# kaiidams/Kokoro-Align

Hardware: NVIDIA B200
Metric: lattice cells/sec (TxS) (higher is better)
Workload: dtype f32

## Files before the change

kokoro-align_b200/csrc/kab_api.cu:

```cuda
#include "../../include/kokoro_align_b200.h"

#include <algorithm>
#include <atomic>
#include <chrono>
#include <map>
#include <mutex>
#include <thread>
#include <unordered_map>
#include <cstdio>
#include <cstdlib>
#include <cstring>
#include <functional>
#include <limits>
#include <new>
#include <optional>
#include <vector>

#include "kab_band.cuh"
#include "kab_bandp.cuh"
#include "kab_bandr.cuh"
#include "kab_btpar.cuh"
#include "kab_wide.cuh"
#include "kab_common.cuh"
#include "kab_compact.cuh"
// ... 195 lines not shown
    if (se.first == stream) ev = se.second;
  if (!ev) {
    KAB_CUDA(cudaEventCreateWithFlags(&ev, cudaEventDisableTiming));
    pl->run_events.emplace_back(stream, ev);
  }
  KAB_CUDA(cudaEventRecord(ev, stream));
  return KAB_OK;
}

void host_teardown(kab_plan *pl) {
  for (kab_plan *c : pl->segs) plan_free(c);
  pl->segs.clear();
  pl->seg_b0.clear();
  for (int k = 0; k < kab_plan::NPIPE; ++k) {
    if (pl->pipe[k]) plan_free(pl->pipe[k]);
    pl->pipe[k] = nullptr;
    pl->pipe_rows[k].clear();
    if (pl->ev_pipe_in[k]) cudaEventDestroy(pl->ev_pipe_in[k]);
    if (pl->ev_pipe_done[k]) cudaEventDestroy(pl->ev_pipe_done[k]);
    if (pl->s_pipe[k]) cudaStreamDestroy(pl->s_pipe[k]);
    pl->ev_pipe_in[k] = nullptr; pl->ev_pipe_done[k] = nullptr; pl->s_pipe[k] = nullptr;
  }
  for (cudaEvent_t e : pl->ev_in) cudaEventDestroy(e);
  for (cudaEvent_t e : pl->ev_cmp) cudaEventDestroy(e);
  pl->ev_in.clear();
  pl->ev_cmp.clear();
  pool_free(pl->d_lp); pool_free(pl->d_path); pool_free(pl->d_lab); pool_free(pl->d_st);
  pool_free(pl->d_sc); pool_free(pl->d_fs); pool_free(pl->d_seg_off); pool_free(pl->d_seg_rec); pool_free(pl->d_lab8);
  pl->d_lp = nullptr; pl->d_path = nullptr; pl->d_lab = nullptr; pl->d_st = nullptr;
  pl->d_sc = nullptr; pl->d_fs = nullptr; pl->d_seg_off = nullptr; pl->d_seg_rec = nullptr; pl->d_lab8 = nullptr;
  pl->seg_cap = 0;
  if (pl->stream) cudaStreamDestroy(pl->stream);
  if (pl->s_in) cudaStreamDestroy(pl->s_in);
  if (pl->s_out) cudaStreamDestroy(pl->s_out);
  pl->stream = nullptr; pl->s_in = nullptr; pl->s_out = nullptr;
  pl->host_ready = false;
}

int plan_free(kab_plan *pl) {
  if (!pl) return KAB_OK;
  Trace tr("kab_plan_destroy");
  DeviceGuard guard;
  guard.enter(pl->device);
  for (auto &se : pl->run_events) {
    cudaEventSynchronize(se.second);
    cudaEventDestroy(se.second);
  }
  pl->run_events.clear();
  if (pl->stream) cudaStreamSynchronize(pl->stream);
  if (pl->s_out) cudaStreamSynchronize(pl->s_out);
  host_teardown(pl);
  if (pl->s_sub) cudaStreamSynchronize(pl->s_sub);
  if (pl->sub) plan_free(pl->sub);
  if (pl->ev_fork) cudaEventDestroy(pl->ev_fork);
  if (pl->ev_join) cudaEventDestroy(pl->ev_join);
  if (pl->s_sub) cudaStreamDestroy(pl->s_sub);
  for (int q = 0; q < N_QUEUES; ++q) pool_free(pl->d_lists[q]);
  pool_free(pl->d_col16); pool_free(pl->d_raw); pool_free(pl->d_bp); pool_free(pl->d_scratch);
  pool_free(pl->d_queue); pool_free(pl->d_status_init); pool_free(pl->d_wide_ws); pool_free(pl->d_band_fifo); pool_free(pl->d_bt_meta); pool_free(pl->d_bt_maps); pool_free(pl->d_bt_entry); pool_free(pl->d_end_state); pool_free(pl->d_gather); pool_free(pl->d_lpc); pool_free(pl->d_nonfinite); pool_free(pl->d_t_off); pool_free(pl->d_seg_scratch); pool_free(pl->d_started);
  delete pl;
  tr.mark("free");
  return KAB_OK;
}

}

extern "C" {

int kab_version(void) { return KAB_VERSION; }

const char *kab_error_string(int code) {
  switch (code) {
    case KAB_OK: return "ok";
    case KAB_E_CUDA: return "CUDA error (see kab_last_cuda_error)";
    case KAB_E_BAD_ARG: return "bad argument";
    case KAB_E_NOMEM: return "out of host memory";
    case KAB_E_UNSUPPORTED: return "unsupported shape";
    default: return "unknown error";
  }
}

const char *kab_last_cuda_error(void) { return g_cuda_err; }

int kab_device_count(int *count) {
  if (!count) return KAB_E_BAD_ARG;
  KAB_CUDA(cudaGetDeviceCount(count));
  return KAB_OK;
}

namespace {
int plan_create_impl(kab_plan **out, int device, const PlanSpec &s, int64_t B, const int64_t *t_off,
                     const int32_t *labels, const int64_t *l_off, const uint8_t *mask, int band_mode);
constexpr int32_t CTC_W = 0x3fffffff, CTC_M = 3;
constexpr int64_t CTC_BAND_MAX_W = 3264;
}

int kab_plan_create(kab_plan **out, int device, int64_t B, const int64_t *t_off, const int32_t *labels,
                    const int64_t *l_off, int32_t V, int32_t W, int32_t M) {
  return plan_create_impl(out, device, PlanSpec{V, W, M}, B, t_off, labels, l_off, nullptr, -1);
}

int kab_plan_create_ctc(kab_plan **out, int device, int64_t B, const int64_t *t_off, const int32_t *labels,
                        const int64_t *l_off, int32_t V, int32_t blank) {
  if (blank < 0 || blank >= V) return KAB_E_BAD_ARG;
  return plan_create_impl(out, device, PlanSpec{V, CTC_W, CTC_M, true, blank}, B, t_off, labels, l_off, nullptr, 0);
}

int kab_plan_create_ctc_long(kab_plan **out, int device, int64_t B, const int64_t *t_off, const int32_t *labels,
                             const int64_t *l_off, int32_t V, int32_t blank) {
  if (blank < 0 || blank >= V) return KAB_E_BAD_ARG;
  return plan_create_impl(out, device, PlanSpec{V, CTC_W, CTC_M, true, blank, true}, B, t_off, labels, l_off, nullptr, 0);
}

int kab_plan_create_ctc_band(kab_plan **out, int device, int64_t B, const int64_t *t_off, const int32_t *labels,
                             const int64_t *l_off, int32_t V, int32_t blank, int32_t beam_size) {
  if (blank < 0 || blank >= V || beam_size < 1) return KAB_E_BAD_ARG;
  return plan_create_impl(out, device, PlanSpec{V, beam_size, CTC_M, true, blank, true}, B, t_off, labels, l_off, nullptr, 0);
}

namespace {

struct Knobs {
  int stage_frames, band_cluster, band_q, band_r, band_hybrid, serial_bt, warp_ctas_per_sm;
  bool band_gather, ctc_compact, serial_setup;
  static int get(const char *name) { const char *v = getenv(name); return v ? atoi(v) : -1; }
  static Knobs read() {
    const char *sb = getenv("KAB_BAND_SERIAL_BT");
    return Knobs{get("KAB_STAGE_FRAMES"), get("KAB_BAND_CLUSTER"), get("KAB_BAND_Q"), get("KAB_BAND_R"), get("KAB_BAND_HYBRID"),
                 sb ? (atoi(sb) != 0) : -1, get("KAB_WARP_CTAS_PER_SM"), get("KAB_BAND_GATHER") != 0, get("KAB_CTC_COMPACT") != 0,
                 getenv("KAB_SERIAL_SETUP") != nullptr};
  }
};

struct LatFacts { uint8_t bad, special, compact; int32_t distinct, repeats; int64_t col_off; };

struct Setup {
  kab_plan *pl;
  const PlanSpec &s;
  const Knobs knob;
  int64_t B;
  const int64_t *t_off, *l_off;
  const int32_t *labels;
  const uint8_t *mask;
  bool gather = false;
  int32_t Veff = 0;
  std::vector<LatFacts> facts;
  std::vector<int32_t> gather_rows;
  std::vector<uint16_t> col16;
  std::vector<int32_t> status_init;
  int64_t bp_bytes = 0, scr_floats = 0, max_band_weff = 0;
  int wide_capacity = 0, wide_max_ctas = 0;
  std::vector<uint8_t> hyb_mask;
  int hyb_k = 0;
  bool in(int64_t b) const { return !mask || mask[b]; }
  int64_t frames(int64_t b) const { return t_off[b + 1] - t_off[b]; }
  int64_t len(int64_t b) const { return l_off[b + 1] - l_off[b]; }
  void for_lattices(const std::function<void(int64_t, int64_t *)> &fn) const;
  void scan_labels(), compact_vocabulary(), classify(), choose_band_kernel(int band_mode), lay_out_band();
  int allocate(), finish();
};

void Setup::for_lattices(const std::function<void(int64_t, int64_t *)> &fn) const {
  const int n_mask = (s.V + 63) / 64;
  const unsigned hw = std::thread::hardware_concurrency();
  const int nt = (B >= 2048 && pl->total_L >= 65536 && hw >= 4 && !knob.serial_setup) ? (int)std::min<unsigned>(8, hw / 2) : 1;
  auto work = [&](int t) {
    std::vector<int64_t> words((size_t)std::max(n_mask, 1), 0);
    const int64_t b0 = B * t / nt, b1 = B * (t + 1) / nt;
    for (int64_t b = b0; b < b1; ++b)
      if (in(b)) fn(b, words.data());
  };
  std::vector<std::thread> th;
  for (int t = 1; t < nt; ++t) th.emplace_back(work, t);
  work(0);
  for (auto &w : th) w.join();
}

void Setup::scan_labels() {
  const int n_mask = (s.V + 63) / 64;
  facts.assign((size_t)B, LatFacts{});
  for_lattices([&](int64_t b, int64_t *seen) {
    const int64_t L = len(b);
    const int32_t *lab = labels + l_off[b];
    LatFacts f{};
    std::fill(seen, seen + n_mask, (int64_t)0);
    for (int64_t l = 0; l < L; ++l) {
      if (s.ctc ? (lab[l] < 0 || lab[l] >= s.V || lab[l] == s.blank) : (lab[l] < -s.V || lab[l] >= s.V)) { f.bad = 1; break; }
      if (!s.ctc && lab[l] <= 0) f.special = 1;
      if (l > 0 && lab[l] == lab[l - 1]) ++f.repeats;
      const int32_t c = lab[l] < 0 ? lab[l] + s.V : lab[l];
      if (!(seen[c >> 6] >> (c & 63) & 1)) { seen[c >> 6] |= (int64_t)1 << (c & 63); ++f.distinct; }
    }
    facts[(size_t)b] = f;
  });
}

void Setup::compact_vocabulary() {
  const int64_t ga_max_weff = (int64_t)KAB_BQ_OW * KAB_BR_CW * 8 - 32;
  bool ok = !s.ctc && s.V > MAX_STAGE_V && s.M <= 4 && knob.band_gather && kab_bandr_geom(64).smem_bytes <= 227 * 1024, any_band = false;
  for (int64_t b = 0; b < B && ok; ++b) {
    const int64_t S = 2 * len(b) + 1;
    if (in(b) && band_shaped(frames(b), S, s.W)) { any_band = true; ok = std::min<int64_t>(s.W, S) <= ga_max_weff; }
  }
  gather = ok && any_band;
  int64_t dmax = -1, off = 0;
  for (int64_t b = 0; b < B; ++b) {
    if (!in(b)) continue;
    LatFacts &f = facts[(size_t)b];
    f.col_off = off;
    if (f.bad) continue;
    off += align_up(len(b), 8) + 8;
    if (f.special || (gather && band_shaped(frames(b), 2 * len(b) + 1, s.W))) continue;
    if (!s.ctc || f.distinct + 1 <= MAX_STAGE_V) dmax = std::max<int64_t>(dmax, f.distinct);
  }
  if (s.V > MAX_STAGE_V && (s.ctc ? knob.ctc_compact : s.M <= 4) && dmax >= 0 && dmax + 1 <= MAX_STAGE_V) {
    pl->Vc = (int32_t)std::max<int64_t>(8, align_up(dmax + 1, 4));
    gather_rows.assign((size_t)B * pl->Vc, 0);
  }
  Veff = pl->Vc ? pl->Vc : s.V;

  pl->stage_frames = Veff <= 64 ? 16 : 8;
  if (knob.stage_frames == 8 || knob.stage_frames == 16 || knob.stage_frames == 32) pl->stage_frames = knob.stage_frames;
  pl->stage_bytes = (int32_t)align_up((int64_t)pl->stage_frames * Veff * 4 + 24, 16);

  col16.assign((size_t)off, 0);
  const int n_mask = (s.V + 63) / 64;
  for_lattices([&](int64_t b, int64_t *seen) {
    LatFacts &f = facts[(size_t)b];
    if (f.bad) return;
    const int64_t L = len(b);
    const int32_t *lab = labels + l_off[b];
    uint16_t *c = col16.data() + f.col_off;
    const bool ga = gather && !f.special && band_shaped(frames(b), 2 * L + 1, s.W);
    if (pl->Vc && !f.special && !ga && f.distinct + 1 <= pl->Vc) {
      f.compact = 1;
      std::fill(seen, seen + n_mask, (int64_t)0);
      for (int64_t l = 0; l < L; ++l) seen[lab[l] >> 6] |= (int64_t)1 << (lab[l] & 63);
      int32_t *g = gather_rows.data() + (size_t)b * pl->Vc;
      g[0] = s.ctc ? s.blank : 0;
      int32_t n = 1;
      for (int w = 0; w < n_mask; ++w)
        for (int64_t m = seen[w]; m; m &= m - 1) g[n++] = w * 64 + __builtin_ctzll((unsigned long long)m);
      for (int64_t l = 0; l < L; ++l) c[l] = (uint16_t)(std::lower_bound(g + 1, g + n, lab[l]) - g);
    } else {
      for (int64_t l = 0; l < L; ++l) c[l] = (uint16_t)(lab[l] < 0 ? lab[l] + s.V : lab[l]);
    }
  });
}

void Setup::classify() {
  const int64_t W = s.W, M = s.M;
  Launch &lw = pl->launch[Q_WIDE];
  lw = Launch{s.ctc ? (const void *)kab_wide_ctc_kernel : (const void *)kab_wide_kernel, dim3(), dim3(KAB_WD_THREADS),
              kab_wide_geom(pl->stage_bytes).smem_bytes, 0, true};
  {
    int occ = 0;
    if (lw.smem <= 227 * 1024 && ensure_dyn_smem(lw.fn, pl->device, lw.smem) == cudaSuccess &&
        cudaOccupancyMaxActiveBlocksPerMultiprocessor(&occ, lw.fn, KAB_WD_THREADS, lw.smem) == cudaSuccess)
      wide_capacity = occ * pl->sm_count;
    (void)cudaGetLastError();
  }
  bool ctc_wide = false;
  if (s.ctc && s.ctc_long) {
    double sum_t = 0.0, cells = 0.0, max_cells = 0.0;
    for (int64_t b = 0; b < B; ++b) {
      if (!in(b) || facts[(size_t)b].bad) continue;
      if (pl->Vc && !facts[(size_t)b].compact) continue;
      const int64_t T = frames(b), S = 2 * len(b) + 1;
      if (!unbanded(T, S, W)) continue;
      if (S + 32 <= KAB_BAND_OW * BAND_MAX_WARPS) continue;
      if (wide_ctas(S) + 1 > wide_capacity) continue;
      sum_t += (double)T;
      cells += (double)T * (double)S;
      max_cells = std::max(max_cells, (double)T * (double)S);
    }
    ctc_wide = sum_t * 102.0 <= std::max(max_cells / 0.68, cells / 79.0);
  }
  kab_plan_info &info = pl->info;
  status_init.assign((size_t)B, 0);
  for (int64_t b = 0; b < B; ++b) {
    if (!in(b)) continue;
    const int64_t T = frames(b), L = len(b), S = 2 * L + 1;
    const LatFacts &f = facts[(size_t)b];
    if (f.bad || (s.ctc && T < L + f.repeats)) {
      status_init[(size_t)b] = f.bad ? KAB_ST_BAD_LABEL : KAB_ST_DEAD_BAND;
      pl->any_bad_label = true;
      continue;
    }
    KabLattice d{};
    d.t_off = t_off[b];
    d.lab_off = l_off[b];
    d.T = (int32_t)T; d.L = (int32_t)L; d.index = (int32_t)b;
    d.col_off = f.col_off;
    const bool ga = gather && !f.special && band_shaped(T, S, W);

    const bool fast = M <= 4 && !f.special && (ga || (Veff <= MAX_STAGE_V && (!pl->Vc || f.distinct + 1 <= pl->Vc)));
    const bool full = unbanded(T, S, W);
    const int64_t weff = std::min<int64_t>(W, S);
    int q;
    if (fast && !ga && full && S <= 248) {
      q = Q_WARP;
      d.k = S <= 62 ? 2 : (S <= 124 ? 4 : (S <= 186 ? 6 : 8));
      d.bp_off = bp_bytes;
      if (s.ctc || d.k <= 4) {
        const int fpw = d.k <= 2 ? 8 : (d.k <= 4 ? 4 : 2);
        bp_bytes += align_up((T + fpw - 1) / fpw * 128, 256);
      } else {
        bp_bytes += align_up((T + KAB_CKPT_C - 1) / KAB_CKPT_C * kab_ckpt_stride((int)S, d.k) * 4, 256);
      }
    } else if (fast && band_shaped(T, S, W) && (!s.ctc || full || weff <= CTC_BAND_MAX_W)) {
      q = Q_BAND;
      max_band_weff = std::max(max_band_weff, weff);
    } else if (fast && !ga && (s.ctc ? ctc_wide : M == 4) && full && wide_ctas(S) + 1 <= wide_capacity) {
      q = Q_WIDE;
      const int nww = (int)((S + KAB_BAND_OW - 1) / KAB_BAND_OW);
      d.k = nww;
      wide_max_ctas = std::max(wide_max_ctas, (int)wide_ctas(S));
      d.bp_off = bp_bytes;
      bp_bytes += (int64_t)nww * ((T + 7) / 8) * 256;
      d.scr_off = pl->wide_ws_bytes / 4;
      pl->wide_ws_bytes += (int64_t)align_up((int64_t)kab_wide_ws_bytes(nww), 256);
    } else {
      q = Q_GENERIC;
      d.bp_off = bp_bytes;
      bp_bytes += align_up(T * std::max<int64_t>(1, weff), 256);
      d.scr_off = scr_floats;
      scr_floats += align_up(2 * (S + 16), 64);
    }
    pl->lists[q].push_back(d);
    pl->max_T[q] = std::max(pl->max_T[q], (int)T);
    info.n_class[q == Q_WARP ? KAB_CLASS_WARP : (q == Q_GENERIC ? KAB_CLASS_GENERIC : (q == Q_WIDE ? KAB_CLASS_WIDE : KAB_CLASS_BAND))]++;
    const int64_t cells = cells_eval_of(T, S, W);
    info.cells_eval += cells;
    info.cells_nominal += T * S;
    int bbits = 0;
    while ((1 << bbits) < M) ++bbits;
    const int64_t dcols = std::min<int64_t>(s.V, f.distinct + 1);
    info.algorithmic_bytes += 4 * dcols * T + (cells * bbits + 7) / 8 + (T * bbits + 7) / 8 + 12 * T;
  }
}

void Setup::choose_band_kernel(int band_mode) {
  std::vector<KabLattice> &bl = pl->lists[Q_BAND];
  if (bl.empty()) return;
  pl->band_nw = (int32_t)((max_band_weff + 32 + KAB_BAND_OW - 1) / KAB_BAND_OW);
  const int nc = (pl->band_nw + KAB_BP_CW - 1) / KAB_BP_CW;
  int want_nc = knob.band_cluster;
  if (band_mode >= 0) want_nc = band_mode == 0 ? 0 : -1;
  const bool cluster_ok = nc <= 8 && kab_bandp_geom(pl->stage_bytes).smem_bytes <= 227 * 1024;
  const int nwq = (int)((max_band_weff + 32 + KAB_BQ_OW - 1) / KAB_BQ_OW);
  const int ncq = (nwq + KAB_BQ_CW - 1) / KAB_BQ_CW;
  const bool q_ok = ncq <= 8 && kab_bandq_geom(pl->stage_bytes).smem_bytes <= 227 * 1024;
  const int ncr = (nwq + KAB_BR_CW - 1) / KAB_BR_CW;
  const bool r_ok = gather || (ncr <= 8 && pl->stage_frames == KAB_BR_F && kab_bandr_geom(pl->stage_bytes).smem_bytes <= 227 * 1024);
  const int want_q = band_mode >= 0 ? (band_mode == 0 ? 0 : -1) : knob.band_q;
  const int want_r = band_mode >= 0 ? band_mode : knob.band_r;
  int64_t n_band = (int64_t)bl.size();
  double sum_t = 0.0, max_t = 0.0, bt_steps = 0.0;
  for (const KabLattice &d : bl) {
    sum_t += d.T; max_t = std::max(max_t, (double)d.T);
    bt_steps += (double)d.T * (double)std::min<int64_t>(s.W, 2 * (int64_t)d.L + 1);
  }
  const double est_r = std::max(max_t * 70.0, sum_t / std::max(1, pl->sm_count / std::max(1, ncr)) * 90.0) + bt_steps * 0.55e-3;
  const double est_b = std::max(max_t, sum_t / (double)(pl->sm_count * (pl->band_nw <= 16 ? 2 : 1))) * 190.0;
  const bool use_r = gather || (r_ok && want_r != 0 && want_nc != 0 && want_q != 0 && (want_r >= 1 || want_nc >= 1 || est_r <= est_b));
  const bool use_q = !use_r && s.M == 4 && q_ok && want_q != 0 && want_nc != 0 && (want_q >= 1 || n_band <= pl->sm_count / ncq);
  const int want_h = knob.band_hybrid;
  if (band_mode < 0 && !mask && !use_r && !use_q && r_ok && !gather && !pl->Vc && s.V <= MAX_STAGE_V && want_h != 0 &&
      want_r < 0 && want_q < 0 && want_nc < 0 && n_band >= 2) {
    std::stable_sort(bl.begin(), bl.end(), [](const KabLattice &a, const KabLattice &b2) { return a.T > b2.T; });
    std::vector<double> pre((size_t)n_band + 1, 0.0);
    for (int64_t i = 0; i < n_band; ++i) pre[(size_t)i + 1] = pre[(size_t)i] + bl[(size_t)i].T;
    const int per_sm = pl->band_nw <= 16 ? 2 : 1;
    double best = est_b;
    int best_k = 0;
    int64_t best_m = 0;
    for (int k = 1; k <= pl->sm_count / ncr / 2; ++k) {
      const double sm_left = (double)(pl->sm_count - k * ncr) * per_sm;
      for (int64_t m = k; m < n_band && m <= 16 * (int64_t)k; ++m) {
        const double tr_ = std::max((double)bl[0].T, pre[(size_t)m] / k) * 70.0;
        const double tb_ = std::max((double)bl[(size_t)m].T, (sum_t - pre[(size_t)m]) / sm_left) * 190.0;
        const double ms = std::max(tr_, tb_);
        if (ms < best) { best = ms; best_k = k; best_m = m; }
      }
    }
    if (want_h >= 1 && best_k == 0) { best_k = 1; best_m = 1; }
    if (best_k > 0 && (want_h >= 1 || best < 0.85 * est_b)) {
      hyb_mask.assign((size_t)B, 0);
      for (int64_t i = 0; i < best_m; ++i) hyb_mask[(size_t)bl[(size_t)i].index] = 1;
      bl.erase(bl.begin(), bl.begin() + best_m);
      hyb_k = best_k;
      want_nc = 0;
      pl->band_sm_reserved = best_k * ncr;
      pl->max_T[Q_BAND] = bl.empty() ? 0 : bl[0].T;
    }
  }
  if (use_r || use_q) {
    pl->band_kernel = use_q ? BandKernel::Q : (gather ? BandKernel::R_GATHER : BandKernel::R);
    pl->band_cw = use_r ? KAB_BR_CW : KAB_BQ_CW; pl->band_nc = use_r ? ncr : ncq;
    return;
  }
  if (want_nc < 0 && cluster_ok) {
    const int64_t resident = pl->sm_count / nc;
    want_nc = (int64_t)bl.size() <= resident ? nc : 0;
  }
  if (s.M == 4 && cluster_ok && want_nc >= 1) {
    pl->band_kernel = BandKernel::P;
    pl->band_cw = KAB_BP_CW; pl->band_nc = std::min(8, std::max(nc, want_nc));
  }
}

bool band_layout_q(BandKernel k) { return k == BandKernel::Q || k == BandKernel::R || k == BandKernel::R_GATHER; }

void Setup::lay_out_band() {
  const BandKernel bk = pl->band_kernel;
  const int nwt = pl->band_cw * pl->band_nc;
  const int nbp = pl->band_nw ? kab_band_geom(pl->band_nw, pl->stage_bytes).nbp : 0;
  for (KabLattice &d : pl->lists[Q_BAND]) {
    d.bp_off = bp_bytes;
    if (bk == BandKernel::CTA) {
      bp_bytes += align_up((int64_t)d.T * nbp, 256);
      continue;
    }
    bp_bytes += (int64_t)((d.T + 7) / 8) * (band_layout_q(bk) ? 128 : 256) * nwt;
    d.scr_off = pl->band_fifo_bytes / 4;
    pl->band_fifo_bytes += (int64_t)align_up((int64_t)(band_layout_q(bk) ? kab_bandq_ws_bytes(nwt) : kab_bandp_ws_bytes(nwt)), 256);
  }
  for (int q = 0; q < N_QUEUES; ++q)
    std::stable_sort(pl->lists[q].begin(), pl->lists[q].end(), [&](const KabLattice &a, const KabLattice &b2) {
      if (q == Q_WARP && a.k != b2.k) return a.k > b2.k;
      return a.T > b2.T;
    });

  if (pl->lists[Q_BAND].empty() || bk == BandKernel::CTA) return;
  if (bk == BandKernel::P) {
    double steps = 0.0, tmax = 0.0;
    for (const KabLattice &d : pl->lists[Q_BAND]) {
      steps += (double)d.T * (double)std::min<int64_t>(s.W, 2 * (int64_t)d.L + 1);
      tmax = std::max(tmax, (double)d.T);
    }
    if (knob.serial_bt >= 0 ? knob.serial_bt != 0 : steps * 0.55e-12 > 0.6 * tmax * 40e-9) return;
  }
  for (const KabLattice &d : pl->lists[Q_BAND]) {
    KabBtMeta m{};
    m.map_off = pl->bt_map_ints;
    m.first_block = pl->bt_blocks;
    m.n_blocks = (d.T + KAB_BT_BLOCK - 1) / KAB_BT_BLOCK;
    m.wl = (int32_t)align_up(std::min<int64_t>(s.W, 2 * (int64_t)d.L + 1), 32);
    pl->bt_map_ints += (int64_t)m.n_blocks * KAB_BT_NSUB * m.wl;
    pl->bt_blocks += m.n_blocks;
    pl->bt_max_wl = std::max(pl->bt_max_wl, m.wl);
    pl->bt_meta.push_back(m);
  }
}

int alloc(void **dst, size_t bytes, const char *what, const void *src = nullptr) {
  cudaError_t e = bytes ? pool_malloc(dst, bytes) : cudaSuccess;
  if (e == cudaSuccess && bytes && src) e = cudaMemcpy(*dst, src, bytes, cudaMemcpyHostToDevice);
  return e == cudaSuccess ? KAB_OK : cuda_fail(e, what);
}

cudaLaunchConfig_t launch_config(const Launch &k, cudaLaunchAttribute *at, cudaStream_t stream) {
  cudaLaunchConfig_t cfg{};
  cfg.gridDim = k.grid; cfg.blockDim = k.block; cfg.dynamicSmemBytes = k.smem; cfg.stream = stream;
  cfg.attrs = at;
  cfg.numAttrs = k.cluster || k.cooperative ? 1 : 0;
  at[0].id = k.cluster ? cudaLaunchAttributeClusterDimension : cudaLaunchAttributeCooperative;
  if (k.cluster) at[0].val.clusterDim = {k.cluster, 1, 1};
  else at[0].val.cooperative = 1;
  return cfg;
}

cudaError_t launch_list(const Launch &k, const KabLattice *lats, int n, KabParams p, unsigned char *const *wide_ws,
                        const int *blank, cudaStream_t stream) {
  void *args[5] = {&lats, &n, &p};
  int na = 3;
  if (wide_ws) args[na++] = (void *)wide_ws;
  if (blank) args[na++] = (void *)blank;
  cudaLaunchAttribute at[1];
  const cudaLaunchConfig_t cfg = launch_config(k, at, stream);
  return cudaLaunchKernelExC(&cfg, k.fn, args);
}

int Setup::allocate() {
  int rc = KAB_OK;
  cudaError_t e;
  for (int q = 0; q < N_QUEUES; ++q)
    if ((rc = alloc((void **)&pl->d_lists[q], pl->lists[q].size() * sizeof(KabLattice), "work list", pl->lists[q].data()))) return rc;
  if ((rc = alloc((void **)&pl->d_col16, col16.size() * sizeof(uint16_t), "column table", col16.data()))) return rc;
  if ((rc = alloc((void **)&pl->d_t_off, B > 0 ? (size_t)(B + 1) * sizeof(int64_t) : 0, "frame offsets", t_off))) return rc;
  if (pl->Vc) {
    if ((rc = alloc((void **)&pl->d_nonfinite, (size_t)B * sizeof(int32_t), "pool_malloc(non-finite flags)"))) return rc;
    if ((rc = alloc((void **)&pl->d_gather, gather_rows.size() * sizeof(int32_t), "gather rows", gather_rows.data()))) return rc;
    if ((rc = alloc((void **)&pl->d_lpc, (size_t)pl->total_T * pl->Vc * sizeof(float), "pool_malloc(compact log-probs)"))) return rc;
  }
  if (!pl->lists[Q_GENERIC].empty() && (rc = alloc((void **)&pl->d_raw, (size_t)pl->total_L * sizeof(int32_t), "labels", labels))) return rc;
  if (pl->any_bad_label && (rc = alloc((void **)&pl->d_status_init, (size_t)B * sizeof(int32_t), "statuses", status_init.data()))) return rc;
  if ((rc = alloc((void **)&pl->d_bp, (size_t)bp_bytes, "pool_malloc(backpointers)"))) return rc;
  if ((rc = alloc((void **)&pl->d_scratch, (size_t)scr_floats * 4, "pool_malloc(scratch)"))) return rc;
  if ((rc = alloc((void **)&pl->d_queue, N_QUEUES * sizeof(unsigned int), "pool_malloc(queue)"))) return rc;
  if (!pl->bt_meta.empty()) {
    if ((rc = alloc((void **)&pl->d_bt_meta, pl->bt_meta.size() * sizeof(KabBtMeta), "backtrack metadata", pl->bt_meta.data()))) return rc;
    if ((rc = alloc((void **)&pl->d_bt_maps, (size_t)pl->bt_map_ints * 4, "pool_malloc(backtrack maps)"))) return rc;
    if ((rc = alloc((void **)&pl->d_bt_entry, (size_t)pl->bt_blocks * 4, "pool_malloc(backtrack entries)"))) return rc;
    if ((rc = alloc((void **)&pl->d_end_state, (size_t)B * 4, "pool_malloc(end states)"))) return rc;
  }
  if ((rc = alloc((void **)&pl->d_band_fifo, (size_t)pl->band_fifo_bytes, "pool_malloc(band FIFOs)"))) return rc;
  if ((rc = alloc((void **)&pl->d_wide_ws, (size_t)pl->wide_ws_bytes, "pool_malloc(wide workspace)"))) return rc;
  if (!pl->lists[Q_WARP].empty()) {
    Launch &l = pl->launch[Q_WARP];
    l.fn = s.ctc ? (const void *)kab_warp_ctc_kernel
         : s.M == 4 ? (Veff == 39 ? (const void *)kab_warp_kernel<39, false> : (const void *)kab_warp_kernel<0, false>)
                    : (Veff == 39 ? (const void *)kab_warp_kernel<39, true> : (const void *)kab_warp_kernel<0, true>);
    l.block = dim3(KAB_WARPS_PER_CTA * 32);
    l.smem = 128 + (size_t)KAB_WARPS_PER_CTA * (KAB_WARP_STAGES * pl->stage_bytes + 256);
    if ((e = ensure_dyn_smem(l.fn, pl->device, l.smem)) != cudaSuccess) return cuda_fail(e, "cudaFuncSetAttribute(warp)");
    int occ = 0;
    if ((e = cudaOccupancyMaxActiveBlocksPerMultiprocessor(&occ, l.fn, l.block.x, l.smem)) != cudaSuccess) return cuda_fail(e, "occupancy(warp)");
    const int64_t ctas = ((int64_t)pl->lists[Q_WARP].size() + KAB_WARPS_PER_CTA - 1) / KAB_WARPS_PER_CTA;
    occ = std::min(occ, KAB_WARP_MINBLOCKS);
    if (knob.warp_ctas_per_sm >= 1) occ = std::min(occ, knob.warp_ctas_per_sm);
    l.grid = dim3((unsigned)std::min<int64_t>(ctas, (int64_t)pl->sm_count * std::max(occ, 1)));
  }
  if (!pl->lists[Q_BAND].empty()) {
    Launch &l = pl->launch[Q_BAND];
    const BandKernel bk = pl->band_kernel;
    const int64_t n_band = (int64_t)pl->lists[Q_BAND].size();
    const bool mm = s.M != 4, small = pl->band_nw <= 16;
    l.fn = bk == BandKernel::P ? (const void *)kab_bandp_kernel
         : bk == BandKernel::Q ? (const void *)kab_bandq_kernel
         : bk == BandKernel::R ? (mm ? (const void *)kab_bandr_kernel<true> : (const void *)kab_bandr_kernel<false>)
         : bk == BandKernel::R_GATHER ? (mm ? (const void *)kab_bandr_kernel<true, true> : (const void *)kab_bandr_kernel<false, true>)
         : s.ctc ? (small ? (const void *)kab_band_ctc_kernel<512> : (const void *)kab_band_ctc_kernel<1024>)
         : small ? (mm ? (const void *)kab_band_kernel<512, true> : (const void *)kab_band_kernel<512, false>)
                 : (mm ? (const void *)kab_band_kernel<1024, true> : (const void *)kab_band_kernel<1024, false>);
    const bool ga = bk == BandKernel::R_GATHER;
    l.stage_frames = ga ? KAB_BR_F : pl->stage_frames;
    l.stage_bytes = ga ? 64 : pl->stage_bytes;
    if (bk == BandKernel::CTA) {
      l.block = dim3(pl->band_nw * 32);
      l.smem = kab_band_geom(pl->band_nw, pl->stage_bytes).smem_bytes;
      int occ = 0;
      if ((e = ensure_dyn_smem(l.fn, pl->device, l.smem)) != cudaSuccess) return cuda_fail(e, "cudaFuncSetAttribute(band)");
      if ((e = cudaOccupancyMaxActiveBlocksPerMultiprocessor(&occ, l.fn, l.block.x, l.smem)) != cudaSuccess) return cuda_fail(e, "occupancy(band)");
      l.grid = dim3((unsigned)std::min<int64_t>(n_band, (int64_t)(pl->sm_count - pl->band_sm_reserved) * std::max(occ, 1)));
    } else {
      const bool r = bk == BandKernel::R || bk == BandKernel::R_GATHER;
      l.block = dim3(r ? KAB_BR_THREADS : (bk == BandKernel::Q ? KAB_BQ_THREADS : KAB_BP_THREADS));
      l.smem = r ? kab_bandr_geom(l.stage_bytes).smem_bytes
                 : (bk == BandKernel::Q ? kab_bandq_geom(l.stage_bytes).smem_bytes : kab_bandp_geom(l.stage_bytes).smem_bytes);
      l.cluster = (unsigned)pl->band_nc;
      if ((e = ensure_dyn_smem(l.fn, pl->device, l.smem)) != cudaSuccess) return cuda_fail(e, "cudaFuncSetAttribute(cluster band)");
      l.grid = dim3((unsigned)(pl->band_nc * pl->sm_count));
      cudaLaunchAttribute at[1];
      const cudaLaunchConfig_t cfg = launch_config(l, at, nullptr);
      int ncl = 0;
      if ((e = cudaOccupancyMaxActiveClusters(&ncl, l.fn, &cfg)) != cudaSuccess) return cuda_fail(e, "cudaOccupancyMaxActiveClusters(cluster band)");
      l.grid = dim3((unsigned)(std::min<int64_t>(std::max(ncl, 1), n_band) * pl->band_nc));
    }
  }
  if (!pl->lists[Q_WIDE].empty()) pl->launch[Q_WIDE].grid = dim3((unsigned)(wide_max_ctas + 1));
  if (!pl->lists[Q_GENERIC].empty())
    pl->launch[Q_GENERIC].grid = dim3((unsigned)std::min<int64_t>((int64_t)pl->lists[Q_GENERIC].size(), (int64_t)pl->sm_count * 4));
  return KAB_OK;
}

int Setup::finish() {
  kab_plan_info &info = pl->info;
  info.backptr_bytes = bp_bytes;
  info.workspace_bytes = bp_bytes + scr_floats * 4 + pl->wide_ws_bytes + pl->band_fifo_bytes + (int64_t)col16.size() * 2 +
                         (pl->d_raw ? pl->total_L * 4 : 0) + B * (int64_t)sizeof(KabLattice);
  info.kernel_launches = 0;
  for (int q = 0; q < N_QUEUES; ++q) info.kernel_launches += pl->lists[q].empty() ? 0 : 1;
  const BandKernel bk = pl->band_kernel;
  if (!pl->lists[Q_BAND].empty()) {
    const int32_t code[] = {KAB_BAND_KERNEL_CTA, KAB_BAND_KERNEL_CLUSTER, KAB_BAND_KERNEL_CLUSTER2, KAB_BAND_KERNEL_SPEC, KAB_BAND_KERNEL_SPEC};
    info.band_kernel = code[(int)bk];
    info.band_cluster = pl->band_nc > 0 ? pl->band_nc : 1;
  }
  if (!pl->bt_meta.empty()) info.kernel_launches += 3;
  if (bk == BandKernel::R || bk == BandKernel::R_GATHER) info.kernel_launches += 1;
  if (pl->Vc)
    for (int q : {Q_WARP, Q_BAND, Q_WIDE}) info.kernel_launches += pl->lists[q].empty() ? 0 : 2;
  if (hyb_k == 0) return KAB_OK;
  if (int rc = plan_create_impl(&pl->sub, pl->device, s, B, t_off, labels, l_off, hyb_mask.data(), 1)) return rc;
  pl->sub->is_child = true;
  pl->sub->launch[Q_BAND].grid.x = std::min(pl->sub->launch[Q_BAND].grid.x, (unsigned)(hyb_k * pl->sub->band_nc));
  cudaError_t e = pool_malloc((void **)&pl->sub->d_started, sizeof(unsigned int));
  if (e == cudaSuccess) e = cudaMemset(pl->sub->d_started, 0, sizeof(unsigned int));
  if (e == cudaSuccess) e = cudaStreamCreateWithFlags(&pl->s_sub, cudaStreamNonBlocking);
  if (e == cudaSuccess) e = cudaEventCreateWithFlags(&pl->ev_fork, cudaEventDisableTiming);
  if (e == cudaSuccess) e = cudaEventCreateWithFlags(&pl->ev_join, cudaEventDisableTiming);
  if (e != cudaSuccess) return cuda_fail(e, "stream / events of the hybrid band plan");
  info.band_kernel = KAB_BAND_KERNEL_HYBRID;
  info.band_cluster = pl->sub->band_nc;
  info.backptr_bytes += pl->sub->info.backptr_bytes;
  info.workspace_bytes += pl->sub->info.workspace_bytes;
  info.kernel_launches += pl->sub->info.kernel_launches;
  return KAB_OK;
}

int plan_create_impl(kab_plan **out, int device, const PlanSpec &s, int64_t B, const int64_t *t_off,
                     const int32_t *labels, const int64_t *l_off, const uint8_t *mask, int band_mode) {
  if (!out || B < 0 || !t_off || !l_off || s.V < 1 || s.V > 65535 || s.W < 0 || s.M < 1 || s.M > 255) return KAB_E_BAD_ARG;
  if (B > 0 && (t_off[0] < 0 || l_off[0] < 0)) return KAB_E_BAD_ARG;
  if (B > 0 && l_off[B] > l_off[0] && !labels) return KAB_E_BAD_ARG;
  for (int64_t b = 0; b < B; ++b) {
// ... 658 lines not shown
```

kokoro-align_b200/csrc/kab_warp.cuh:

```cuda
#pragma once
#include "kab_common.cuh"

#define KAB_WARP_STAGES 3
#define KAB_WARPS_PER_CTA 4
#ifndef KAB_WARP_MINBLOCKS
#define KAB_WARP_MINBLOCKS 6
#endif

#define KAB_CKPT_C 8

__host__ __device__ inline int kab_ckpt_stride(int S, int K) { return (K * ((S + K - 1) / K) + 3) & ~3; }

template <int K>
struct KabWarpCfg {
  static constexpr int BPF = K <= 2 ? 4 : (K <= 4 ? 8 : 16);
  static constexpr int FPW = 32 / BPF;
};

template <int K, bool MM>
__device__ __forceinline__ void kab_warp_frame(float (&s)[K], const float eb, const float (&el)[K / 2],
                                               const bool lane1, const float mm1, const float mm2, const float mm3) {
  float h1, h2, h3;
  if (K >= 4) {
    h1 = __shfl_up_sync(KAB_FULL_MASK, s[K - 1], 1);
    h2 = __shfl_up_sync(KAB_FULL_MASK, s[K - 2], 1);
    h3 = __shfl_up_sync(KAB_FULL_MASK, s[K >= 4 ? K - 3 : 0], 1);
  } else {
    h1 = __shfl_up_sync(KAB_FULL_MASK, s[1], 1);
    h2 = __shfl_up_sync(KAB_FULL_MASK, s[0], 1);
    h3 = __shfl_up_sync(KAB_FULL_MASK, s[1], 2);
    h3 = lane1 ? kab_neg_inf() : h3;
  }
  float n[K];
#pragma unroll
  for (int q = 0; q < K / 2; ++q) {
    const int kb = 2 * q, kl = 2 * q + 1;
    const float b1 = kb >= 1 ? s[kb >= 1 ? kb - 1 : 0] : h1;
    const float b3 = kb >= 3 ? s[kb >= 3 ? kb - 3 : 0] : (kb == 2 ? h1 : h3);
    const float mb = kab_max3(s[kb], kab_mm<MM>(b1, mm1), kab_mm<MM>(b3, mm3));
    const float l2 = q >= 1 ? s[q >= 1 ? kl - 2 : 0] : h1;
    const float l3 = q >= 1 ? s[q >= 1 ? kl - 3 : 0] : h2;
    const float ml = kab_max3(kab_max2(s[kl], kab_mm<MM>(s[kl - 1], mm1)), kab_mm<MM>(l2, mm2), kab_mm<MM>(l3, mm3));
    kab_add2v(mb, ml, eb, el[q], n[kb], n[kl]);
  }
#pragma unroll
  for (int k = 0; k < K; ++k) s[k] = n[k];
}

template <int K, bool MM>
__device__ __forceinline__ void kab_warp_frame_bp(float (&s)[K], const float eb, const float (&el)[K / 2],
                                               const bool lane1, uint32_t &w, const int shift,
                                                  const uint32_t one, const float mm1, const float mm2, const float mm3) {
  float h1, h2, h3;
  if (K >= 4) {
    h1 = __shfl_up_sync(KAB_FULL_MASK, s[K - 1], 1);
    h2 = __shfl_up_sync(KAB_FULL_MASK, s[K - 2], 1);
    h3 = __shfl_up_sync(KAB_FULL_MASK, s[K >= 4 ? K - 3 : 0], 1);
  } else {
    h1 = __shfl_up_sync(KAB_FULL_MASK, s[1], 1);
    h2 = __shfl_up_sync(KAB_FULL_MASK, s[0], 1);
    h3 = __shfl_up_sync(KAB_FULL_MASK, s[1], 2);
    h3 = lane1 ? kab_neg_inf() : h3;
  }
  float t[K];
#pragma unroll
  for (int m = 0; m < K / 2; ++m) kab_add2(s[2 * m], s[2 * m + 1], eb, t[2 * m], t[2 * m + 1]);
  const float th1 = __fadd_rn(h1, eb), th3 = __fadd_rn(h3, eb);
  float n[K];
#pragma unroll
  for (int q = 0; q < K / 2; ++q) {
    const int kb = 2 * q, kl = 2 * q + 1;
    const float b1 = kb >= 1 ? t[kb >= 1 ? kb - 1 : 0] : th1;
    const float b3 = kb >= 3 ? t[kb >= 3 ? kb - 3 : 0] : (kb == 2 ? th1 : th3);
    n[kb] = kab_blank_sel(t[kb], kab_mm<MM>(b1, mm1), kab_mm<MM>(b3, mm3), w, 1u << (shift + 2 * kb), 2u << (shift + 2 * kb), one);
    float a0, a1, a2, a3;
    kab_add2(s[kl - 1], s[kl], el[q], a1, a0);
    if (q >= 1) kab_add2(s[q >= 1 ? kl - 3 : 0], s[q >= 1 ? kl - 2 : 0], el[q], a3, a2);
    else kab_add2(h2, h1, el[q], a3, a2);
    n[kl] = kab_label_sel(a0, kab_mm<MM>(a1, mm1), kab_mm<MM>(a2, mm2), kab_mm<MM>(a3, mm3), w, 1u << (shift + 2 * kl), 2u << (shift + 2 * kl), one);
  }
#pragma unroll
  for (int k = 0; k < K; ++k) s[k] = n[k];
}

template <int K>
__device__ __forceinline__ void kab_ckpt_store(float *row, const float (&s)[K]) {
  if (K % 4 == 0) {
#pragma unroll
    for (int k = 0; k < K; k += 4)
      __stcg(reinterpret_cast<float4 *>(row + k), make_float4(s[k], s[k + 1], s[k + 2], s[k + 3]));
  } else {
#pragma unroll
    for (int k = 0; k < K; k += 2) __stcg(reinterpret_cast<float2 *>(row + k), make_float2(s[k], s[k + 1]));
  }
}

template <int K>
__device__ __forceinline__ void kab_warp_frame_ctc(float (&s)[K], const float eb, const float (&el)[K / 2],
                                                   const uint32_t rep, uint32_t &w, const int shift) {
  const float h1 = __shfl_up_sync(KAB_FULL_MASK, s[K - 1], 1);
  float n[K];
#pragma unroll
  for (int q = 0; q < K / 2; ++q) {
    const int kb = 2 * q, kl = 2 * q + 1;
    n[kb] = __fadd_rn(kab_ctc_blank_sel(s[kb], kb >= 1 ? s[kb >= 1 ? kb - 1 : 0] : h1, w, shift + 2 * kb), eb);
    const float x2 = (rep >> q) & 1u ? kab_neg_inf() : (kl >= 3 ? s[kl >= 3 ? kl - 2 : 0] : h1);
    n[kl] = __fadd_rn(kab_ctc_label_sel(s[kl], s[kl - 1], x2, w, shift + 2 * kl), el[q]);
  }
#pragma unroll
  for (int k = 0; k < K; ++k) s[k] = n[k];
}

template <int K, int VCT, bool MM, bool CTC>
__device__ void kab_warp_align(const KabLattice &lat, const KabParams &p, float *stage_base, uint64_t *bars,
                               uint16_t *labtab, const uint64_t policy, uint32_t &chunk_counter, const int lane,
                               const int blank) {
  using Cfg = KabWarpCfg<K>;
  constexpr int BPF = Cfg::BPF, FPW = Cfg::FPW;
  constexpr int C = KAB_CKPT_C;
  constexpr bool BP = CTC || K <= 4;
  const int T = lat.T, S = 2 * lat.L + 1;
  const int V = VCT ? VCT : p.V;
  const int F = p.stage_frames;
  const uint32_t stage_words = p.stage_bytes >> 2;
  const int n_chunks = (T + F - 1) / F;
  const uint16_t *col16 = p.col16 + lat.col_off;
  uint32_t *bpw = reinterpret_cast<uint32_t *>(p.bp + lat.bp_off);
  float *ck = reinterpret_cast<float *>(p.bp + lat.bp_off);
  const int RS = kab_ckpt_stride(S, K);
  const bool lane0 = lane == 0, lane1 = lane == 1;
  const uint32_t one = p.one;
  const float mm1 = p.mm1, mm2 = p.mm2, mm3 = p.mm3;
  const int sbase = K * (lane - 1);

  uint32_t coff[K / 2];
  uint32_t rep = 0;
#pragma unroll
  for (int q = 0; q < K / 2; ++q) {
    const int v = sbase + 2 * q + 1;
    const uint32_t col = (v > 0 && v < S) ? col16[(v - 1) >> 1] : 0u;
    coff[q] = 4u * col;
    if (v > 0 && v < S) labtab[(v - 1) >> 1] = (uint16_t)col;
    if (CTC && (v < 3 || v >= S || col == col16[(v - 3) >> 1])) rep |= 1u << q;
  }
  const uint32_t boff = CTC ? 4u * (uint32_t)blank : 0u;

  float s[K];
#pragma unroll
  for (int k = 0; k < K; ++k) s[k] = kab_neg_inf();
  if (lane1) s[0] = 0.0f;

  const uint32_t cc0 = chunk_counter;
  const int64_t lat_b0 = lat.t_off * (int64_t)V * 4;
  const char *lp_base = reinterpret_cast<const char *>(p.lp) + (lat_b0 & ~(int64_t)15);
  const int w0 = (int)((lat_b0 & 15) >> 2);
  const uint32_t chunk_stride = (uint32_t)(F * V * 4);
  const uint32_t full_bytes = (chunk_stride + (uint32_t)w0 * 4u + 15u) & ~15u;
  uint32_t ist = cc0 % KAB_WARP_STAGES;
  auto issue = [&](int c) {
    float *dst = stage_base + ist * stage_words;
    if (c + 1 < n_chunks) {
      if (lane0) {
        kab_mbar_expect_tx(&bars[ist], full_bytes);
        kab_bulk_g2s_hint(dst, lp_base + (size_t)c * chunk_stride, full_bytes, &bars[ist], policy);
      }
    } else {
      const int f0 = c * F;
      const KabStageDesc d = kab_stage_desc(p, lat.t_off, f0, T - f0);
      if (lane0) {
        kab_mbar_expect_tx(&bars[ist], d.bytes);
        if (d.bytes) kab_bulk_g2s_hint(dst, d.src, d.bytes, &bars[ist], policy);
      }
      if (lane < (int)d.tail_n)
        dst[d.tail_word + lane] = __ldg(reinterpret_cast<const float *>(d.src) + d.tail_word + lane);
    }
    ist = ist + 1 == KAB_WARP_STAGES ? 0 : ist + 1;
  };
  const int pre = min(n_chunks, KAB_WARP_STAGES - 1);
  for (int c = 0; c < pre; ++c) issue(c);

  float poison = kab_poison_init<CTC>();
  uint32_t *bprow = bpw + lane;
  float *ckrow = ck;
  uint32_t st = cc0 % KAB_WARP_STAGES, ph = (cc0 / KAB_WARP_STAGES) & 1u;
  for (int c = 0; c < n_chunks; ++c) {
    __syncwarp();
    if (c + KAB_WARP_STAGES - 1 < n_chunks) issue(c + KAB_WARP_STAGES - 1);
    kab_mbar_wait(&bars[st], ph);
    __syncwarp();
    const int nf = min(F, T - c * F);
    const float *stage = stage_base + st * stage_words;
    if (++st == KAB_WARP_STAGES) { st = 0; ph ^= 1u; }
    const int w1 = w0 + nf * V;
    {
      const int v0 = (w0 + 3) >> 2, v1 = w1 >> 2;
      const float4 *s4 = reinterpret_cast<const float4 *>(stage);
      for (int j = v0 + lane; j < v1; j += 32) {
        const float4 x = s4[j];
        poison = kab_poison_t<CTC>(kab_poison_t<CTC>(kab_poison_t<CTC>(kab_poison_t<CTC>(poison, x.x), x.y), x.z), x.w);
      }
      if (lane < 4 * v0 - w0 && w0 + lane < w1) poison = kab_poison_t<CTC>(poison, stage[w0 + lane]);
      if (4 * v1 >= w0 && lane < w1 - 4 * v1) poison = kab_poison_t<CTC>(poison, stage[4 * v1 + lane]);
    }
    const char *rowb = reinterpret_cast<const char *>(stage + w0);
    if constexpr (BP) {
      const int n_groups = nf / FPW;
      for (int gi = 0; gi < n_groups; ++gi, rowb += FPW * V * 4) {
        uint32_t word = 0;
#pragma unroll
        for (int f = 0; f < FPW; ++f) {
          const char *rb = rowb + f * V * 4;
          const float eb = *reinterpret_cast<const float *>(rb + boff);
          float el[K / 2];
#pragma unroll
          for (int q = 0; q < K / 2; ++q) el[q] = *reinterpret_cast<const float *>(rb + coff[q]);
          if (CTC) kab_warp_frame_ctc<K>(s, eb, el, rep, word, f * BPF);
          else kab_warp_frame_bp<K, MM>(s, eb, el, lane1, word, f * BPF, one, mm1, mm2, mm3);
        }
        *bprow = word;
        bprow += 32;
      }
      const int rem = nf - n_groups * FPW;
      if (rem) {
        uint32_t word = 0;
#pragma unroll 1
        for (int f = 0; f < rem; ++f, rowb += V * 4) {
          const float eb = *reinterpret_cast<const float *>(rowb + boff);
          float el[K / 2];
#pragma unroll
          for (int q = 0; q < K / 2; ++q) el[q] = *reinterpret_cast<const float *>(rowb + coff[q]);
          uint32_t fw = 0;
          if (CTC) kab_warp_frame_ctc<K>(s, eb, el, rep, fw, 0);
          else kab_warp_frame_bp<K, MM>(s, eb, el, lane1, fw, 0, one, mm1, mm2, mm3);
          word |= fw << (f * BPF);
        }
        *bprow = word;
      }
    } else {
      const int n_groups = nf / C;
      for (int gi = 0; gi < n_groups; ++gi, rowb += C * V * 4) {
#pragma unroll
        for (int f = 0; f < C; ++f) {
          const char *rb = rowb + f * V * 4;
          const float eb = *reinterpret_cast<const float *>(rb);
          float el[K / 2];
#pragma unroll
          for (int q = 0; q < K / 2; ++q) el[q] = *reinterpret_cast<const float *>(rb + coff[q]);
          kab_warp_frame<K, MM>(s, eb, el, lane1, mm1, mm2, mm3);
        }
        if (!lane0 && sbase < S) kab_ckpt_store<K>(ckrow + sbase, s);
        ckrow += RS;
      }
      const int rem = nf - n_groups * C;
#pragma unroll 1
      for (int f = 0; f < rem; ++f, rowb += V * 4) {
        const float eb = *reinterpret_cast<const float *>(rowb);
        float el[K / 2];
#pragma unroll
        for (int q = 0; q < K / 2; ++q) el[q] = *reinterpret_cast<const float *>(rowb + coff[q]);
        kab_warp_frame<K, MM>(s, eb, el, lane1, mm1, mm2, mm3);
      }
    }
  }
  chunk_counter = cc0 + n_chunks;
  __syncwarp();

  auto score_of = [&](int u) {
    float mine = s[0];
#pragma unroll
    for (int k = 1; k < K; ++k) if (k == u % K) mine = s[k];
    return __shfl_sync(KAB_FULL_MASK, mine, u / K + 1);
  };
  int v;
  if (CTC) {
    v = S - 1;
    if (S >= 2) {
      const float a1 = score_of(S - 1), a2 = score_of(S - 2);
      if (!(a1 > a2)) v = S - 2;
    }
  } else {
    int cand = -1;
#pragma unroll
    for (int k = 0; k < K; ++k) {
      const int v = sbase + k;
      if (v >= 0 && v < S && s[k] > kab_neg_inf()) cand = v;
    }
    v = __reduce_max_sync(KAB_FULL_MASK, cand);
  }
  const bool any_bad = __any_sync(KAB_FULL_MASK, poison != poison);
  const int status = any_bad ? 3 : (v < 0 ? 1 : 0);
  {
    float fs = __int_as_float(0x7fc00000);
    if (status == 0) {
      float mine = s[0];
#pragma unroll
      for (int k = 1; k < K; ++k) if (k == v % K) mine = s[k];
      fs = __shfl_sync(KAB_FULL_MASK, mine, v / K + 1);
    }
    if (lane0) {
      p.status[lat.index] = status;
      if (p.final_score) p.final_score[lat.index] = fs;
    }
  }
  if (status != 0) return;
  if constexpr (!BP) {
    int32_t *out_path = p.best_path + lat.t_off;
    int32_t *out_lab = p.best_labels + lat.t_off;
    float *out_sc = p.best_scores + lat.t_off;
    int ve = v;
    auto win_load = [&](int row, int sb, float &r0, float &r1) {
      const float *rp = ck + (size_t)max(row, 0) * RS;
      r0 = __ldcg(rp + max(sb + lane, 0));
      r1 = __ldcg(rp + max(sb + 32 + lane, 0));
    };
    int sb = ve - 63;
    float r0, r1;
    win_load((T - 1) / C - 1, sb, r0, r1);
    for (int k = 0; k < pre; ++k) issue(n_chunks - 1 - k);
    for (int k = 0; k < n_chunks; ++k) {
      const int c = n_chunks - 1 - k;
      __syncwarp();
      if (k + KAB_WARP_STAGES - 1 < n_chunks) issue(c - (KAB_WARP_STAGES - 1));
      kab_mbar_wait(&bars[st], ph);
      __syncwarp();
      const int nf = min(F, T - c * F);
      const char *rows = reinterpret_cast<const char *>(stage_base + st * stage_words + w0);
      if (++st == KAB_WARP_STAGES) { st = 0; ph ^= 1u; }
      for (int bi = (nf - 1) / C; bi >= 0; --bi) {
        const int f0 = c * F + bi * C, n = min(C, nf - bi * C);
        const char *rb = rows + bi * C * V * 4;
        const int base = ve - 3 * C;
        const int wi = base + lane - sb;
        const float x0 = __shfl_sync(KAB_FULL_MASK, r0, wi & 31), x1 = __shfl_sync(KAB_FULL_MASK, r1, wi & 31);
        const int u = base + lane;
        float x = u < 0 ? kab_neg_inf() : (wi >= 32 ? x1 : x0);
        if (f0 == 0) x = u == 0 ? 0.0f : kab_neg_inf();
        sb = ve - 63;
        win_load(f0 / C - 2, sb, r0, r1);
        const bool blank_lane = (u & 1) == 0;
        const uint32_t uoff = (u > 0 && u < S && !blank_lane) ? 4u * labtab[(u - 1) >> 1] : 0u;
        uint32_t cw = 0;
#pragma unroll
        for (int j = 0; j < C; ++j) {
          const float e = *reinterpret_cast<const float *>(rb + j * V * 4 + uoff);
          const float h1 = __shfl_up_sync(KAB_FULL_MASK, x, 1);
          const float h2 = __shfl_up_sync(KAB_FULL_MASK, x, 2);
          const float h3 = __shfl_up_sync(KAB_FULL_MASK, x, 3);
          float a0, a1, a2, a3;
          kab_add2(x, h1, e, a0, a1);
          kab_add2(h2, h3, e, a2, a3);
          a2 = blank_lane ? kab_neg_inf() : kab_mm<MM>(a2, mm2);
          x = kab_label_sel(a0, kab_mm<MM>(a1, mm1), a2, kab_mm<MM>(a3, mm3), cw, 1u << (2 * j), 2u << (2 * j), one);
        }
        if (n < C) cw &= (1u << (2 * n)) - 1u;
        int wl = 3 * C;
        uint32_t mw = 0;
#pragma unroll
        for (int j = C - 1; j >= 0; --j) {
          const uint32_t w = __shfl_sync(KAB_FULL_MASK, cw, wl);
          mw |= w & (3u << (2 * j));
          wl -= (int)((w >> (2 * j)) & 3u);
        }
        const uint32_t above = mw >> min(2 * lane + 2, 2 * C);
        const int myv = ve - (__popc(above & 0x55555555u) + 2 * __popc(above & 0xaaaaaaaau));
        ve = base + wl;
        if (lane < n) {
          const int lab = (myv & 1) ? (int)labtab[(myv - 1) >> 1] : 0;
          out_path[f0 + lane] = myv;
          out_lab[f0 + lane] = lab;
          out_sc[f0 + lane] = *reinterpret_cast<const float *>(rb + lane * V * 4 + lab * 4);
        }
      }
    }
    chunk_counter += n_chunks;
  } else {
    constexpr int RB = 4;
    int32_t *out_path = p.best_path + lat.t_off;
    int32_t *out_lab = p.best_labels + lat.t_off;
    float *out_sc = p.best_scores + lat.t_off;
    const float *lp = p.lp + lat.t_off * (int64_t)V;
    const int n_rows = (T + FPW - 1) / FPW;
    auto fetch = [&](int rb, uint32_t (&w)[RB]) {
#pragma unroll
      for (int r = 0; r < RB; ++r)
        w[r] = (rb >= 0 && (rb + r) < n_rows) ? __ldcg(&bpw[(size_t)(rb + r) * 32 + lane]) : 0u;
    };
    int myv = 0, pend_t = -1;
    float pend_s = 0.0f;
    int own1 = v / K + 1, k2 = 2 * (v - (v / K) * K);
    uint32_t wr[RB], wn[RB];
    const int rb_last = ((n_rows - 1) / RB) * RB;
    fetch(rb_last, wr);
    for (int rb = rb_last; rb >= 0; rb -= RB) {
      fetch(rb - RB, wn);
      const int fb = rb * FPW;
      const int lb = lane - (fb & 31);
#pragma unroll
      for (int r = RB - 1; r >= 0; --r) {
#pragma unroll
        for (int f = FPW - 1; f >= 0; --f) {
          const uint32_t w = __shfl_sync(KAB_FULL_MASK, wr[r], own1);
          if (lb == r * FPW + f) myv = v;
          const int mv = (int)((w >> (f * BPF + k2)) & 3u);
          v -= mv;
          k2 -= 2 * mv;
          if (k2 < 0) { k2 += 2 * K; --own1; }
          if (K == 2 && k2 < 0) { k2 += 2 * K; --own1; }
        }
      }
      if ((fb & 31) == 0) {
        if (pend_t >= 0) out_sc[pend_t] = pend_s;
        const int t = fb + lane;
        pend_t = -1;
        if (t < T) {
          const int lab = (myv & 1) ? (int)labtab[(myv - 1) >> 1] : (CTC ? blank : 0);
          out_path[t] = myv;
          out_lab[t] = lab;
          pend_s = __ldg(&lp[(int64_t)t * V + lab]);
          pend_t = t;
        }
      }
#pragma unroll
      for (int r = 0; r < RB; ++r) wr[r] = wn[r];
    }
    if (pend_t >= 0) out_sc[pend_t] = pend_s;
  }
}

template <int VCT, bool MM, bool CTC>
__device__ __forceinline__ void kab_warp_body(const KabLattice *__restrict__ lats, int n_lat, const KabParams &p,
                                              const int blank) {
  extern __shared__ __align__(128) unsigned char kab_smem[];
  const int warp = threadIdx.x >> 5, lane = threadIdx.x & 31;
  uint64_t *bars = reinterpret_cast<uint64_t *>(kab_smem) + warp * KAB_WARP_STAGES;
  float *stage_base = reinterpret_cast<float *>(kab_smem + 128 +
                                                (size_t)warp * KAB_WARP_STAGES * p.stage_bytes);
  uint16_t *labtab = reinterpret_cast<uint16_t *>(kab_smem + 128 +
                                                  (size_t)KAB_WARPS_PER_CTA * KAB_WARP_STAGES * p.stage_bytes) +
                     warp * 128;
  uint64_t policy;
  asm volatile("createpolicy.fractional.L2::evict_normal.b64 %0, 1.0;" : "=l"(policy));
  if (lane == 0) {
    for (int s = 0; s < KAB_WARP_STAGES; ++s) kab_mbar_init(&bars[s], 1);
    kab_fence_mbar_init();
  }
  __syncwarp();
  uint32_t chunk_counter = 0;
  for (;;) {
    unsigned int item = 0;
    if (lane == 0) item = atomicAdd(p.queue, 1u);
    item = __shfl_sync(KAB_FULL_MASK, item, 0);
    if (item >= (unsigned int)n_lat) break;
    const KabLattice lat = lats[item];
    switch (lat.k) {
      case 2: kab_warp_align<2, VCT, MM, CTC>(lat, p, stage_base, bars, labtab, policy, chunk_counter, lane, blank); break;
      case 4: kab_warp_align<4, VCT, MM, CTC>(lat, p, stage_base, bars, labtab, policy, chunk_counter, lane, blank); break;
      case 6: kab_warp_align<6, VCT, MM, CTC>(lat, p, stage_base, bars, labtab, policy, chunk_counter, lane, blank); break;
      default: kab_warp_align<8, VCT, MM, CTC>(lat, p, stage_base, bars, labtab, policy, chunk_counter, lane, blank); break;
    }
    __syncwarp();
  }
}

template <int VCT, bool MM>
__global__ void __launch_bounds__(KAB_WARPS_PER_CTA * 32, KAB_WARP_MINBLOCKS)
    kab_warp_kernel(const KabLattice *__restrict__ lats, int n_lat, KabParams p) {
  kab_warp_body<VCT, MM, false>(lats, n_lat, p, 0);
}

__global__ void __launch_bounds__(KAB_WARPS_PER_CTA * 32, KAB_WARP_MINBLOCKS)
    kab_warp_ctc_kernel(const KabLattice *__restrict__ lats, int n_lat, KabParams p, int blank) {
  kab_warp_body<0, false, true>(lats, n_lat, p, blank);
}
```

Baseline: 1723 billion.

## Use checkpoint recomputation instead of per-frame backpointers for small non-CTC warp lattices

Non-CTC warp-path lattices with K<=4 now take the checkpoint path (store the state every 8 frames and recompute during backtrace) instead of emitting 2-bit backpointers every frame. The specialised non-CTC backpointer frame function is removed and buffer sizing is changed to match. This trims select/bit-packing work in the forward loop, but the backtrace now has to recompute frames and checkpoint storage per lattice grows.

New measurement: 1743 billion, median of 6. +1.2%, better.

```diff
diff --git a/kokoro-align_b200/csrc/kab_api.cu b/kokoro-align_b200/csrc/kab_api.cu
--- a/kokoro-align_b200/csrc/kab_api.cu
+++ b/kokoro-align_b200/csrc/kab_api.cu
@@ -521,7 +521,7 @@
       q = Q_WARP;
       d.k = S <= 62 ? 2 : (S <= 124 ? 4 : (S <= 186 ? 6 : 8));
       d.bp_off = bp_bytes;
-      if (s.ctc || d.k <= 4) {
+      if (s.ctc) {
         const int fpw = d.k <= 2 ? 8 : (d.k <= 4 ? 4 : 2);
         bp_bytes += align_up((T + fpw - 1) / fpw * 128, 256);
       } else {
diff --git a/kokoro-align_b200/csrc/kab_warp.cuh b/kokoro-align_b200/csrc/kab_warp.cuh
--- a/kokoro-align_b200/csrc/kab_warp.cuh
+++ b/kokoro-align_b200/csrc/kab_warp.cuh
@@ -47,42 +47,6 @@
   for (int k = 0; k < K; ++k) s[k] = n[k];
 }
 
-template <int K, bool MM>
-__device__ __forceinline__ void kab_warp_frame_bp(float (&s)[K], const float eb, const float (&el)[K / 2],
-                                               const bool lane1, uint32_t &w, const int shift,
-                                                  const uint32_t one, const float mm1, const float mm2, const float mm3) {
-  float h1, h2, h3;
-  if (K >= 4) {
-    h1 = __shfl_up_sync(KAB_FULL_MASK, s[K - 1], 1);
-    h2 = __shfl_up_sync(KAB_FULL_MASK, s[K - 2], 1);
-    h3 = __shfl_up_sync(KAB_FULL_MASK, s[K >= 4 ? K - 3 : 0], 1);
-  } else {
-    h1 = __shfl_up_sync(KAB_FULL_MASK, s[1], 1);
-    h2 = __shfl_up_sync(KAB_FULL_MASK, s[0], 1);
-    h3 = __shfl_up_sync(KAB_FULL_MASK, s[1], 2);
-    h3 = lane1 ? kab_neg_inf() : h3;
-  }
-  float t[K];
-#pragma unroll
-  for (int m = 0; m < K / 2; ++m) kab_add2(s[2 * m], s[2 * m + 1], eb, t[2 * m], t[2 * m + 1]);
-  const float th1 = __fadd_rn(h1, eb), th3 = __fadd_rn(h3, eb);
-  float n[K];
-#pragma unroll
-  for (int q = 0; q < K / 2; ++q) {
-    const int kb = 2 * q, kl = 2 * q + 1;
-    const float b1 = kb >= 1 ? t[kb >= 1 ? kb - 1 : 0] : th1;
-    const float b3 = kb >= 3 ? t[kb >= 3 ? kb - 3 : 0] : (kb == 2 ? th1 : th3);
-    n[kb] = kab_blank_sel(t[kb], kab_mm<MM>(b1, mm1), kab_mm<MM>(b3, mm3), w, 1u << (shift + 2 * kb), 2u << (shift + 2 * kb), one);
-    float a0, a1, a2, a3;
-    kab_add2(s[kl - 1], s[kl], el[q], a1, a0);
-    if (q >= 1) kab_add2(s[q >= 1 ? kl - 3 : 0], s[q >= 1 ? kl - 2 : 0], el[q], a3, a2);
-    else kab_add2(h2, h1, el[q], a3, a2);
-    n[kl] = kab_label_sel(a0, kab_mm<MM>(a1, mm1), kab_mm<MM>(a2, mm2), kab_mm<MM>(a3, mm3), w, 1u << (shift + 2 * kl), 2u << (shift + 2 * kl), one);
-  }
-#pragma unroll
-  for (int k = 0; k < K; ++k) s[k] = n[k];
-}
-
 template <int K>
 __device__ __forceinline__ void kab_ckpt_store(float *row, const float (&s)[K]) {
   if (K % 4 == 0) {
@@ -118,7 +82,7 @@
   using Cfg = KabWarpCfg<K>;
   constexpr int BPF = Cfg::BPF, FPW = Cfg::FPW;
   constexpr int C = KAB_CKPT_C;
-  constexpr bool BP = CTC || K <= 4;
+  constexpr bool BP = CTC;
   const int T = lat.T, S = 2 * lat.L + 1;
   const int V = VCT ? VCT : p.V;
   const int F = p.stage_frames;
@@ -214,8 +178,7 @@
           float el[K / 2];
 #pragma unroll
           for (int q = 0; q < K / 2; ++q) el[q] = *reinterpret_cast<const float *>(rb + coff[q]);
-          if (CTC) kab_warp_frame_ctc<K>(s, eb, el, rep, word, f * BPF);
-          else kab_warp_frame_bp<K, MM>(s, eb, el, lane1, word, f * BPF, one, mm1, mm2, mm3);
+          kab_warp_frame_ctc<K>(s, eb, el, rep, word, f * BPF);
         }
         *bprow = word;
         bprow += 32;
@@ -230,8 +193,7 @@
 #pragma unroll
           for (int q = 0; q < K / 2; ++q) el[q] = *reinterpret_cast<const float *>(rowb + coff[q]);
           uint32_t fw = 0;
-          if (CTC) kab_warp_frame_ctc<K>(s, eb, el, rep, fw, 0);
-          else kab_warp_frame_bp<K, MM>(s, eb, el, lane1, fw, 0, one, mm1, mm2, mm3);
+          kab_warp_frame_ctc<K>(s, eb, el, rep, fw, 0);
           word |= fw << (f * BPF);
         }
         *bprow = word;
```
